# GPUOpen-Effects/FidelityFX-FSR

Hardware: NVIDIA H100
Metric: upscaled Mpixels/sec (EASU+RCAS) (higher is better)
Workload: dtype f16

## Files before the change

### fidelityfx-fsr_b200/csrc/fsr1_fused.cu

```cuda
#include "fsr1_easu_quad.cuh"
#include "fsr1_post.cuh"
#include "fsr1_rcas_math.cuh"

namespace fsr1 {

constexpr int kFBW = kQBW + 2;
constexpr int kFSW = kFBW - 2;
constexpr int kStripCells = 31;

struct FusedParams {
  ImgView in, out;
  int y0, y1;
  uint32_t sharp_h2;
  int n_strips;
  HaloSync sync = {};
};

template <int NW> struct FusedCfg {
  static constexpr int kCY = 2 * NW, kBH = kCY + 3, kSH = kCY + 1, kElems = kFBW * kBH;
  static constexpr int kPad = ((kElems * 8 + 127) / 128) * 128 / 8;
  static constexpr int kMidRows = 2 * kCY + 2;
};

template <int NW> struct __align__(128) FusedSmem {
  uint2 tile[2][FusedCfg<NW>::kPad];
  float4 S[kFSW * FusedCfg<NW>::kSH];
  uint4 mid[FusedCfg<NW>::kMidRows][32];
  float L[FusedCfg<NW>::kElems];
  uint64_t bar[2];
};

template <bool kIn> struct MidSink {
  uint4* top;
  bool zT, zB;
  uint32_t keep;
  __device__ __forceinline__ void put(bool bottom, __half2 oR, __half2 oG, __half2 oB) const {
    if (kIn) {
      top[bottom ? 32 : 0] = make_uint4(h22u(oR), h22u(oG), h22u(oB), 0u);
      return;
    }
    const uint32_t m = (bottom ? zB : zT) ? 0u : keep;
    top[bottom ? 32 : 0] = make_uint4(h22u(oR) & m, h22u(oG) & m, h22u(oB) & m, 0u);
  }
};

struct FusedStep { int tx, m0, n, ya, yb; };

template <int CY> struct FusedIter {
  int y0, y1, mfirst, mlast;
  int strip, strip_end, ma, mb, m;
  __device__ void init(const FusedParams& p, int cta, int ctas) {
    y0 = p.y0; y1 = p.y1;
    mfirst = (y0 - 2) >> 1;
    mlast = (y1 - 1) >> 1;
    const int S = p.n_strips, C = mlast - mfirst + 1;
    strip = strip_end = 0; ma = 0; mb = -1; m = 1;
    if (y1 <= y0) return;
    if (ctas < S) {
      strip = (int)((long long)S * cta / ctas);
      strip_end = (int)((long long)S * (cta + 1) / ctas);
      ma = mfirst; mb = mlast; m = ma;
      return;
    }
    const int s = (int)(((long long)(cta + 1) * S - 1) / ctas);
    const int g0 = (int)((long long)ctas * s / S), g = (int)((long long)ctas * (s + 1) / S) - g0, i = cta - g0;
    int T = (C + g - 1 + CY - 1) / CY;
    if (T < g) T = (C - 1 + CY - 2) / (CY - 1);
    const int a = (int)((long long)T * i / g), k = (int)((long long)T * (i + 1) / g) - a;
    const int ra = mfirst + CY * a - (i < a ? i : a);
    if (k == 0 || 2 * ra + 2 >= y1) return;
    ma = ra;
    mb = ma + CY * k - 1 < mlast ? ma + CY * k - 1 : mlast;
    strip = s; strip_end = s + 1; m = ma;
  }
  __device__ bool next(FusedStep& s) {
    if (m > mb) {
      if (++strip >= strip_end) return false;
      m = ma;
    }
    s.tx = strip; s.m0 = m;
    s.ya = 2 * ma + 2 > y0 ? 2 * ma + 2 : y0;
    s.yb = 2 * mb + 2 < y1 ? 2 * mb + 2 : y1;
    s.n = mb - m + 1 < CY ? mb - m + 1 : CY;
    m += s.n;
    return true;
  }
};

template <bool kIn, int NW, typename SO>
__device__ __forceinline__ void fused_step(FusedSmem<NW>& sm, const FusedParams& p, const FusedStep& cur, const uint2* tile, int dx,
                                           int k0, __half2 sharp, int lane, int warp, const PostParams* q) {
  constexpr int CY = FusedCfg<NW>::kCY;
  constexpr bool kPost = !std::is_void<SO>::value;
  const int n = cur.n;
#pragma unroll 1
  for (int q = 0; q < 2; q++) {
    const int r = warp + q * NW;
    if (!kIn && r >= n) break;
    const int pyT = 2 * (cur.m0 + r) + 1, pxA = 2 * (k0 + lane) + 1;
    MidSink<kIn> sink;
    sink.top = &sm.mid[2 * r + 2][lane];
    sink.zT = !kIn && (pyT < 0 || pyT >= p.out.h);
    sink.zB = !kIn && (pyT + 1 < 0 || pyT + 1 >= p.out.h);
    sink.keep = kIn ? 0xffffffffu
                    : ((pxA >= 0 && pxA < p.out.w) ? 0x0000ffffu : 0u) | ((pxA + 1 >= 0 && pxA + 1 < p.out.w) ? 0xffff0000u : 0u);
    quad_compute<MidSink<kIn>, kFBW, kFSW>(tile + dx, sm.S + dx, lane, r, true, true, sink);
  }
  __syncthreads();
  constexpr int kR = 2 * CY / NW;
  const int o_first = 2 * cur.m0 + warp * kR;
  const int i0 = warp * kR;
  const int lm = lane > 0 ? lane - 1 : 0;
  const int ox = 2 * (k0 + lane);
  const bool writer = lane >= 1 && (kIn || ox < p.out.w);
  const bool wtop = writer && (!kIn || o_first >= cur.ya);
  if constexpr (kPost) {
    auto mid_row = [&](int i, Row3& e, Row3& d, Row3& f) {
      const uint4 a = sm.mid[i][lm], c = sm.mid[i][lane];
      e.r = uh2(__byte_perm(a.x, c.x, 0x5432));
      e.g = uh2(__byte_perm(a.y, c.y, 0x5432));
      e.b = uh2(__byte_perm(a.z, c.z, 0x5432));
      d.r = uh2(a.x); d.g = uh2(a.y); d.b = uh2(a.z);
      f.r = uh2(c.x); f.g = uh2(c.y); f.b = uh2(c.z);
    };
    Row3 ea, eb, db, fb, ec, dc, fc;
    mid_row(i0, ea, dc, fc);
    mid_row(i0 + 1, eb, db, fb);
    unsigned char* dst = p.out.base + (long long)(o_first - p.out.row0) * p.out.pitch + (long long)ox * PostStore<SO>::kBytes;
    PostCursor pc;
    pc.init(*q, ox, o_first);
#pragma unroll
    for (int r = 0; r < kR; r++) {
      const int o = o_first + r;
      mid_row(i0 + r + 2, ec, dc, fc);
      if (kIn || (o >= cur.ya && o < cur.yb && o < 2 * cur.m0 + 2 * n)) {
        __half2 oR, oG, oB;
        rcas_pair<0>(ea, db, eb, fb, ec, sharp, oR, oG, oB);
        if (r >= 2 ? writer : wtop) post_pair<SO>(*q, pc, dst + (long long)r * p.out.pitch, ox, o, oR, oG, oB, 0x3c003c00u, kIn || ox + 1 < p.out.w);
      }
      pc.next_row(*q);
      ea = eb; eb = ec; db = dc; fb = fc;
    }
  } else {
    Row3 E[kR + 2], D[kR], Fv[kR];
#pragma unroll
    for (int r = 0; r < kR + 2; r++) {
      const uint4 a = sm.mid[i0 + r][lm], c = sm.mid[i0 + r][lane];
      E[r].r = uh2(__byte_perm(a.x, c.x, 0x5432));
      E[r].g = uh2(__byte_perm(a.y, c.y, 0x5432));
      E[r].b = uh2(__byte_perm(a.z, c.z, 0x5432));
      if (r >= 1 && r <= kR) {
        D[r - 1].r = uh2(a.x); D[r - 1].g = uh2(a.y); D[r - 1].b = uh2(a.z);
        Fv[r - 1].r = uh2(c.x); Fv[r - 1].g = uh2(c.y); Fv[r - 1].b = uh2(c.z);
      }
    }
    unsigned char* dst = p.out.base + (long long)(o_first - p.out.row0) * p.out.pitch + (long long)ox * 8;
#pragma unroll
    for (int r = 0; r < kR; r++) {
      const int o = o_first + r;
      if (kIn || (o >= cur.ya && o < cur.yb && o < 2 * cur.m0 + 2 * n)) {
        __half2 oR, oG, oB;
        rcas_pair<0>(E[r], D[r], E[r + 1], Fv[r], E[r + 2], sharp, oR, oG, oB);
        if (r >= 2 ? writer : wtop) {
          const uint4 w = pack_pair_half(oR, oG, oB, 0x3c003c00u);
          unsigned char* o8 = dst + (long long)r * p.out.pitch;
          if (kIn || ox + 1 < p.out.w) *reinterpret_cast<uint4*>(o8) = w;
          else *reinterpret_cast<uint2*>(o8) = make_uint2(w.x, w.y);
        }
      }
    }
  }
}

template <int NW, typename SO, bool kSrtmIn>
__device__ __forceinline__ void fused_body(const FusedParams p, const CUtensorMap& tmap, const PostParams* q) {
  using C = FusedCfg<NW>;
  constexpr int NT = NW * 32, CY = C::kCY;
  __shared__ FusedSmem<NW> sm;
  const int tid = threadIdx.x, lane = tid & 31, warp = tid >> 5;
  if (tid == 0) {
    mbar_init(&sm.bar[0], 1);
    mbar_init(&sm.bar[1], 1);
    mbar_fence_init();
  }
  __syncthreads();
  halo_sync_begin(p.sync);
  FusedIter<CY> iter;
  iter.init(p, blockIdx.x, gridDim.x);
  FusedStep cur, nxt;
  bool has = iter.next(cur);
  auto box_x = [](const FusedStep& s) { return (kStripCells * s.tx - 2) & ~1; };
  if (tid == 0 && has) {
    mbar_expect_tx(&sm.bar[0], C::kElems * 8u);
    tma_load_2d(sm.tile[0], &tmap, box_x(cur), cur.m0 - 1 - p.in.row0, &sm.bar[0]);
  }
  const __half2 sharp = uh2(p.sharp_h2);
  for (int it = 0; has; it++) {
    const int b = it & 1;
    const bool hasn = iter.next(nxt);
    if (tid == 0 && hasn) {
      fence_proxy_async();
      mbar_expect_tx(&sm.bar[b ^ 1], C::kElems * 8u);
      tma_load_2d(sm.tile[b ^ 1], &tmap, box_x(nxt), nxt.m0 - 1 - p.in.row0, &sm.bar[b ^ 1]);
    }
    uint2* tile = sm.tile[b];
    const int k0 = kStripCells * cur.tx - 1;
    const int gxe = box_x(cur), dx = (k0 - 1) - gxe;
    const int gy0 = cur.m0 - 1, n = cur.n;
    mbar_wait(&sm.bar[b], (it >> 1) & 1);
    if (gxe < 0 || gy0 < 0 || gxe + kFBW > p.in.w || gy0 + C::kBH > p.in.h) {
      clamp_fixup(tile, kFBW, kFBW, C::kBH, gxe, gy0, p.in.w, p.in.h, lane, warp, NW);
      fence_proxy_async();
      __syncthreads();
    }
    for (int i = tid; i < kFBW * (n + 3); i += NT) {
      uint2 c = tile[i];
      if (kSrtmIn) tile[i] = c = srtm_texel(c);
      sm.L[i] = texel_luma(c);
    }
    __syncthreads();
    for (int idx = tid; idx < kFSW * (n + 1); idx += NT) {
      const int j = idx / kFSW, i = idx - j * kFSW;
      const float* c = sm.L + (j + 1) * kFBW + (i + 1);
      sm.S[idx] = texel_terms(c[-kFBW], c[-1], c[0], c[1], c[kFBW]);
    }
    __syncthreads();
    const bool inside = k0 >= 0 && 2 * (k0 + 31) + 2 < p.out.w && cur.m0 >= 0 && 2 * (cur.m0 + CY) < p.out.h && n == CY &&
                        2 * cur.m0 + 2 >= cur.ya && 2 * (cur.m0 + CY) <= cur.yb;
    if (inside) fused_step<true, NW, SO>(sm, p, cur, tile, dx, k0, sharp, lane, warp, q);
    else fused_step<false, NW, SO>(sm, p, cur, tile, dx, k0, sharp, lane, warp, q);
    __syncthreads();
    if (n == CY && tid < 64) {
      const int rr = tid >> 5;
      sm.mid[rr][lane] = sm.mid[2 * CY + rr][lane];
    }
    cur = nxt;
    has = hasn;
  }
  halo_sync_end(p.sync);
}

template <int NW, int MINB, bool kSrtmIn = false>
__global__ void __launch_bounds__(NW * 32, MINB)
fused_h_quad2x_kernel(const FusedParams p, const __grid_constant__ CUtensorMap tmap) {
  fused_body<NW, void, kSrtmIn>(p, tmap, nullptr);
}

template <int NW, int MINB, typename SO, bool kSrtmIn = false>
__global__ void __launch_bounds__(NW * 32, MINB)
fused_h_quad2x_post_kernel(const FusedParams p, const __grid_constant__ CUtensorMap tmap, const __grid_constant__ PostParams q) {
  fused_body<NW, SO, kSrtmIn>(p, tmap, &q);
}

#ifndef FSR1_CPU_EMU
static cudaError_t fused_setup(const EasuParams& e, uint32_t sharp_h2, int out_align, CUtensorMap& tmap, FusedParams& p, int& per_sm,
                               long long& grid) {
  if (!(e.c0x == 0.5f && e.c0y == 0.5f && e.c0z == -0.25f && e.c0w == -0.25f)) return cudaErrorNotSupported;
  if ((reinterpret_cast<uintptr_t>(e.in.base) & 15) || (e.in.pitch & 15) || (reinterpret_cast<uintptr_t>(e.out.base) & (out_align - 1)) ||
      (e.out.pitch & (out_align - 1)))
    return cudaErrorNotSupported;
  constexpr int NW = 4;
  using C = FusedCfg<NW>;
  EncodeTiledFn encode = get_encode_fn();
  if (!encode) return cudaErrorNotSupported;
  const cuuint64_t dims[2] = {(cuuint64_t)e.in.w, (cuuint64_t)e.in.rows};
  const cuuint64_t strides[1] = {(cuuint64_t)e.in.pitch};
  const cuuint32_t box[2] = {(cuuint32_t)kFBW, (cuuint32_t)C::kBH};
  const cuuint32_t estr[2] = {1, 1};
  if (encode(&tmap, CU_TENSOR_MAP_DATA_TYPE_UINT64, 2, e.in.base, dims, strides, box, estr, CU_TENSOR_MAP_INTERLEAVE_NONE,
             CU_TENSOR_MAP_SWIZZLE_NONE, CU_TENSOR_MAP_L2_PROMOTION_L2_128B, CU_TENSOR_MAP_FLOAT_OOB_FILL_NONE) != CUDA_SUCCESS)
    return cudaErrorNotSupported;
  p.in = e.in; p.out = e.out; p.y0 = e.y0; p.y1 = e.y1; p.sharp_h2 = sharp_h2; p.sync = e.sync;
  p.n_strips = ((e.out.w + 1) / 2 + kStripCells - 1) / kStripCells;
  const long long units = (long long)p.n_strips * ((e.y1 - e.y0 + 1) / 2);
  if (p.sync.ready[0] || p.sync.ready[1]) per_sm = 6;
  grid = (long long)per_sm * sm_count();
  if (grid > (units + 7) / 8) grid = (units + 7) / 8;
  if (grid < 1) grid = 1;
  return cudaSuccess;
}

cudaError_t launch_fused_h(const EasuParams& e, uint32_t sharp_h2, int clamp, cudaStream_t s, const char** name, bool srtm_in) {
  if (clamp) return cudaErrorNotSupported;
  CUtensorMap tmap;
  FusedParams p;
  int per_sm = 7;
  long long grid = 0;
  const cudaError_t err = fused_setup(e, sharp_h2, 16, tmap, p, per_sm, grid);
  if (err != cudaSuccess) return err;
  if (srtm_in) {
    fused_h_quad2x_kernel<4, 7, true><<<(int)grid, 4 * 32, 0, s>>>(p, tmap);
    *name = per_sm == 7 ? "fused_easu_rcas_h_quad2x<4w,7/sm,tma2,strips,srtm_in>" : "fused_easu_rcas_h_quad2x<4w,6/sm,tma2,strips,srtm_in>";
  } else {
    fused_h_quad2x_kernel<4, 7><<<(int)grid, 4 * 32, 0, s>>>(p, tmap);
    *name = per_sm == 7 ? "fused_easu_rcas_h_quad2x<4w,7/sm,tma2,strips>" : "fused_easu_rcas_h_quad2x<4w,6/sm,tma2,strips>";
  }
  return cudaGetLastError();
}

constexpr int kPostPerSm = 6;

cudaError_t launch_fused_h_post(const EasuParams& e, uint32_t sharp_h2, const PostParams& q, int out_format, cudaStream_t s,
                                const char** name, bool srtm_in) {
  CUtensorMap tmap;
  FusedParams p;
  int per_sm = kPostPerSm;
  long long grid = 0;
  const cudaError_t err = fused_setup(e, sharp_h2, out_format == 1 ? 16 : 8, tmap, p, per_sm, grid);
  if (err != cudaSuccess) return err;
  switch (out_format * 2 + (srtm_in ? 1 : 0)) {
    case 2:
      fused_h_quad2x_post_kernel<4, kPostPerSm, __half><<<(int)grid, 4 * 32, 0, s>>>(p, tmap, q);
      *name = "fused_easu_rcas_h_quad2x<4w,6/sm,tma2,strips,post,rgba16f>";
      break;
    case 6:
      fused_h_quad2x_post_kernel<4, kPostPerSm, Unorm8><<<(int)grid, 4 * 32, 0, s>>>(p, tmap, q);
      *name = "fused_easu_rcas_h_quad2x<4w,6/sm,tma2,strips,post,rgba8>";
      break;
    case 8:
      fused_h_quad2x_post_kernel<4, kPostPerSm, Unorm10><<<(int)grid, 4 * 32, 0, s>>>(p, tmap, q);
      *name = "fused_easu_rcas_h_quad2x<4w,6/sm,tma2,strips,post,rgb10a2>";
      break;
    case 3:
      fused_h_quad2x_post_kernel<4, kPostPerSm, __half, true><<<(int)grid, 4 * 32, 0, s>>>(p, tmap, q);
      *name = "fused_easu_rcas_h_quad2x<4w,6/sm,tma2,strips,post,rgba16f,srtm_in>";
      break;
    case 7:
      fused_h_quad2x_post_kernel<4, kPostPerSm, Unorm8, true><<<(int)grid, 4 * 32, 0, s>>>(p, tmap, q);
      *name = "fused_easu_rcas_h_quad2x<4w,6/sm,tma2,strips,post,rgba8,srtm_in>";
      break;
    case 9:
      fused_h_quad2x_post_kernel<4, kPostPerSm, Unorm10, true><<<(int)grid, 4 * 32, 0, s>>>(p, tmap, q);
      *name = "fused_easu_rcas_h_quad2x<4w,6/sm,tma2,strips,post,rgb10a2,srtm_in>";
      break;
    default: return cudaErrorNotSupported;
  }
  return cudaGetLastError();
}
#endif

}
```

Before: 105,600.

## Raise fused EASU+RCAS tile height to three cell rows per warp

Makes the number of cell rows each warp handles a template parameter, set by default to three instead of two, so each CTA tile covers more output rows and the vertical halo (loads, luma and terms rows) is amortized over more work. The RCAS output loop is unified into a single rolling-row form, with a reduced unroll for the post-processing path. The launches now request the maximum shared-memory carveout so the larger tiles still fit 7 (or 6) CTAs per SM, and static asserts check this. The cost is more shared memory and longer per-step work per CTA, which may reduce load balance or occupancy.

```diff
diff --git a/fidelityfx-fsr_b200/csrc/fsr1_fused.cu b/fidelityfx-fsr_b200/csrc/fsr1_fused.cu
--- a/fidelityfx-fsr_b200/csrc/fsr1_fused.cu
+++ b/fidelityfx-fsr_b200/csrc/fsr1_fused.cu
@@ -5,8 +5,9 @@
 namespace fsr1 {
 
 constexpr int kFBW = kQBW + 2;
-constexpr int kFSW = kFBW - 2;
+constexpr int kFSW = 34;
 constexpr int kStripCells = 31;
+constexpr int kFusedCPW = 3;
 
 struct FusedParams {
   ImgView in, out;
@@ -16,17 +17,18 @@
   HaloSync sync = {};
 };
 
-template <int NW> struct FusedCfg {
-  static constexpr int kCY = 2 * NW, kBH = kCY + 3, kSH = kCY + 1, kElems = kFBW * kBH;
+template <int NW, int CPW = kFusedCPW> struct FusedCfg {
+  static constexpr int kCY = CPW * NW, kBH = kCY + 3, kSH = kCY + 1, kElems = kFBW * kBH;
   static constexpr int kPad = ((kElems * 8 + 127) / 128) * 128 / 8;
   static constexpr int kMidRows = 2 * kCY + 2;
 };
 
-template <int NW> struct __align__(128) FusedSmem {
-  uint2 tile[2][FusedCfg<NW>::kPad];
-  float4 S[kFSW * FusedCfg<NW>::kSH];
-  uint4 mid[FusedCfg<NW>::kMidRows][32];
-  float L[FusedCfg<NW>::kElems];
+template <int NW, int CPW> struct __align__(128) FusedSmem {
+  using C = FusedCfg<NW, CPW>;
+  uint2 tile[2][C::kPad];
+  float4 S[kFSW * C::kSH];
+  uint4 mid[C::kMidRows][32];
+  float L[C::kElems];
   uint64_t bar[2];
 };
 
@@ -87,14 +89,13 @@
   }
 };
 
-template <bool kIn, int NW, typename SO>
-__device__ __forceinline__ void fused_step(FusedSmem<NW>& sm, const FusedParams& p, const FusedStep& cur, const uint2* tile, int dx,
+template <bool kIn, int NW, int CPW, typename SO>
+__device__ __forceinline__ void fused_step(FusedSmem<NW, CPW>& sm, const FusedParams& p, const FusedStep& cur, const uint2* tile, int dx,
                                            int k0, __half2 sharp, int lane, int warp, const PostParams* q) {
-  constexpr int CY = FusedCfg<NW>::kCY;
   constexpr bool kPost = !std::is_void<SO>::value;
   const int n = cur.n;
 #pragma unroll 1
-  for (int q = 0; q < 2; q++) {
+  for (int q = 0; q < CPW; q++) {
     const int r = warp + q * NW;
     if (!kIn && r >= n) break;
     const int pyT = 2 * (cur.m0 + r) + 1, pxA = 2 * (k0 + lane) + 1;
@@ -107,76 +108,56 @@
     quad_compute<MidSink<kIn>, kFBW, kFSW>(tile + dx, sm.S + dx, lane, r, true, true, sink);
   }
   __syncthreads();
-  constexpr int kR = 2 * CY / NW;
+  constexpr int kR = 2 * CPW;
   const int o_first = 2 * cur.m0 + warp * kR;
   const int i0 = warp * kR;
   const int lm = lane > 0 ? lane - 1 : 0;
   const int ox = 2 * (k0 + lane);
   const bool writer = lane >= 1 && (kIn || ox < p.out.w);
   const bool wtop = writer && (!kIn || o_first >= cur.ya);
-  if constexpr (kPost) {
-    auto mid_row = [&](int i, Row3& e, Row3& d, Row3& f) {
-      const uint4 a = sm.mid[i][lm], c = sm.mid[i][lane];
-      e.r = uh2(__byte_perm(a.x, c.x, 0x5432));
-      e.g = uh2(__byte_perm(a.y, c.y, 0x5432));
-      e.b = uh2(__byte_perm(a.z, c.z, 0x5432));
-      d.r = uh2(a.x); d.g = uh2(a.y); d.b = uh2(a.z);
-      f.r = uh2(c.x); f.g = uh2(c.y); f.b = uh2(c.z);
-    };
-    Row3 ea, eb, db, fb, ec, dc, fc;
-    mid_row(i0, ea, dc, fc);
-    mid_row(i0 + 1, eb, db, fb);
-    unsigned char* dst = p.out.base + (long long)(o_first - p.out.row0) * p.out.pitch + (long long)ox * PostStore<SO>::kBytes;
-    PostCursor pc;
-    pc.init(*q, ox, o_first);
-#pragma unroll
-    for (int r = 0; r < kR; r++) {
-      const int o = o_first + r;
-      mid_row(i0 + r + 2, ec, dc, fc);
-      if (kIn || (o >= cur.ya && o < cur.yb && o < 2 * cur.m0 + 2 * n)) {
-        __half2 oR, oG, oB;
-        rcas_pair<0>(ea, db, eb, fb, ec, sharp, oR, oG, oB);
-        if (r >= 2 ? writer : wtop) post_pair<SO>(*q, pc, dst + (long long)r * p.out.pitch, ox, o, oR, oG, oB, 0x3c003c00u, kIn || ox + 1 < p.out.w);
-      }
-      pc.next_row(*q);
-      ea = eb; eb = ec; db = dc; fb = fc;
-    }
-  } else {
-    Row3 E[kR + 2], D[kR], Fv[kR];
-#pragma unroll
-    for (int r = 0; r < kR + 2; r++) {
-      const uint4 a = sm.mid[i0 + r][lm], c = sm.mid[i0 + r][lane];
-      E[r].r = uh2(__byte_perm(a.x, c.x, 0x5432));
-      E[r].g = uh2(__byte_perm(a.y, c.y, 0x5432));
-      E[r].b = uh2(__byte_perm(a.z, c.z, 0x5432));
-      if (r >= 1 && r <= kR) {
-        D[r - 1].r = uh2(a.x); D[r - 1].g = uh2(a.y); D[r - 1].b = uh2(a.z);
-        Fv[r - 1].r = uh2(c.x); Fv[r - 1].g = uh2(c.y); Fv[r - 1].b = uh2(c.z);
-      }
-    }
-    unsigned char* dst = p.out.base + (long long)(o_first - p.out.row0) * p.out.pitch + (long long)ox * 8;
-#pragma unroll
-    for (int r = 0; r < kR; r++) {
-      const int o = o_first + r;
-      if (kIn || (o >= cur.ya && o < cur.yb && o < 2 * cur.m0 + 2 * n)) {
-        __half2 oR, oG, oB;
-        rcas_pair<0>(E[r], D[r], E[r + 1], Fv[r], E[r + 2], sharp, oR, oG, oB);
-        if (r >= 2 ? writer : wtop) {
+  auto mid_row = [&](int i, Row3& e, Row3& d, Row3& f) {
+    const uint4 a = sm.mid[i][lm], c = sm.mid[i][lane];
+    e.r = uh2(__byte_perm(a.x, c.x, 0x5432));
+    e.g = uh2(__byte_perm(a.y, c.y, 0x5432));
+    e.b = uh2(__byte_perm(a.z, c.z, 0x5432));
+    d.r = uh2(a.x); d.g = uh2(a.y); d.b = uh2(a.z);
+    f.r = uh2(c.x); f.g = uh2(c.y); f.b = uh2(c.z);
+  };
+  Row3 ea, eb, db, fb, ec, dc, fc;
+  mid_row(i0, ea, dc, fc);
+  mid_row(i0 + 1, eb, db, fb);
+  unsigned char* dst = p.out.base + (long long)(o_first - p.out.row0) * p.out.pitch + (long long)ox * PostStore<SO>::kBytes;
+  PostCursor pc;
+  if constexpr (kPost) pc.init(*q, ox, o_first);
+  constexpr int kUnroll = kPost ? 2 : kR;
+#pragma unroll kUnroll
+  for (int r = 0; r < kR; r++) {
+    const int o = o_first + r;
+    mid_row(i0 + r + 2, ec, dc, fc);
+    if (kIn || (o >= cur.ya && o < cur.yb && o < 2 * cur.m0 + 2 * n)) {
+      __half2 oR, oG, oB;
+      rcas_pair<0>(ea, db, eb, fb, ec, sharp, oR, oG, oB);
+      if (r >= 2 ? writer : wtop) {
+        unsigned char* o8 = dst + (long long)r * p.out.pitch;
+        if constexpr (kPost) {
+          post_pair<SO>(*q, pc, o8, ox, o, oR, oG, oB, 0x3c003c00u, kIn || ox + 1 < p.out.w);
+        } else {
           const uint4 w = pack_pair_half(oR, oG, oB, 0x3c003c00u);
-          unsigned char* o8 = dst + (long long)r * p.out.pitch;
           if (kIn || ox + 1 < p.out.w) *reinterpret_cast<uint4*>(o8) = w;
           else *reinterpret_cast<uint2*>(o8) = make_uint2(w.x, w.y);
         }
       }
     }
-  }
-}
-
-template <int NW, typename SO, bool kSrtmIn>
+    if constexpr (kPost) pc.next_row(*q);
+    ea = eb; eb = ec; db = dc; fb = fc;
+  }
+}
+
+template <int NW, int CPW, typename SO, bool kSrtmIn>
 __device__ __forceinline__ void fused_body(const FusedParams p, const CUtensorMap& tmap, const PostParams* q) {
-  using C = FusedCfg<NW>;
+  using C = FusedCfg<NW, CPW>;
   constexpr int NT = NW * 32, CY = C::kCY;
-  __shared__ FusedSmem<NW> sm;
+  __shared__ FusedSmem<NW, CPW> sm;
   const int tid = threadIdx.x, lane = tid & 31, warp = tid >> 5;
   if (tid == 0) {
     mbar_init(&sm.bar[0], 1);
@@ -227,8 +208,8 @@
     __syncthreads();
     const bool inside = k0 >= 0 && 2 * (k0 + 31) + 2 < p.out.w && cur.m0 >= 0 && 2 * (cur.m0 + CY) < p.out.h && n == CY &&
                         2 * cur.m0 + 2 >= cur.ya && 2 * (cur.m0 + CY) <= cur.yb;
-    if (inside) fused_step<true, NW, SO>(sm, p, cur, tile, dx, k0, sharp, lane, warp, q);
-    else fused_step<false, NW, SO>(sm, p, cur, tile, dx, k0, sharp, lane, warp, q);
+    if (inside) fused_step<true, NW, CPW, SO>(sm, p, cur, tile, dx, k0, sharp, lane, warp, q);
+    else fused_step<false, NW, CPW, SO>(sm, p, cur, tile, dx, k0, sharp, lane, warp, q);
     __syncthreads();
     if (n == CY && tid < 64) {
       const int rr = tid >> 5;
@@ -240,19 +221,42 @@
   halo_sync_end(p.sync);
 }
 
-template <int NW, int MINB, bool kSrtmIn = false>
+template <int NW, int MINB, bool kSrtmIn = false, int CPW = kFusedCPW>
 __global__ void __launch_bounds__(NW * 32, MINB)
 fused_h_quad2x_kernel(const FusedParams p, const __grid_constant__ CUtensorMap tmap) {
-  fused_body<NW, void, kSrtmIn>(p, tmap, nullptr);
-}
-
-template <int NW, int MINB, typename SO, bool kSrtmIn = false>
+  fused_body<NW, CPW, void, kSrtmIn>(p, tmap, nullptr);
+}
+
+template <int NW, int MINB, typename SO, bool kSrtmIn = false, int CPW = kFusedCPW>
 __global__ void __launch_bounds__(NW * 32, MINB)
 fused_h_quad2x_post_kernel(const FusedParams p, const __grid_constant__ CUtensorMap tmap, const __grid_constant__ PostParams q) {
-  fused_body<NW, SO, kSrtmIn>(p, tmap, &q);
+  fused_body<NW, CPW, SO, kSrtmIn>(p, tmap, &q);
 }
 
 #ifndef FSR1_CPU_EMU
+constexpr int kPostPerSm = 6;
+
+constexpr size_t kFusedSmemPerCta = sizeof(FusedSmem<4, kFusedCPW>) + 1024;
+static_assert(7 * kFusedSmemPerCta <= 228 * 1024, "the fused kernel's shared memory must admit 7 CTAs per SM");
+static_assert(kPostPerSm * kFusedSmemPerCta <= 228 * 1024, "the fused post kernels' shared memory must admit 6 CTAs per SM");
+
+template <auto K> static cudaError_t max_shared_carveout() {
+  static bool done[64] = {};
+  int dev = 0;
+  if (cudaGetDevice(&dev) != cudaSuccess || dev < 0 || dev >= 64) dev = -1;
+  if (dev >= 0 && done[dev]) return cudaSuccess;
+  const cudaError_t e = cudaFuncSetAttribute(K, cudaFuncAttributePreferredSharedMemoryCarveout, (int)cudaSharedmemCarveoutMaxShared);
+  if (e == cudaSuccess && dev >= 0) done[dev] = true;
+  return e;
+}
+
+template <auto K, typename... A> static cudaError_t fused_launch(long long grid, cudaStream_t s, const A&... args) {
+  const cudaError_t e = max_shared_carveout<K>();
+  if (e != cudaSuccess) return e;
+  K<<<(int)grid, 4 * 32, 0, s>>>(args...);
+  return cudaGetLastError();
+}
+
 static cudaError_t fused_setup(const EasuParams& e, uint32_t sharp_h2, int out_align, CUtensorMap& tmap, FusedParams& p, int& per_sm,
                                long long& grid) {
   if (!(e.c0x == 0.5f && e.c0y == 0.5f && e.c0z == -0.25f && e.c0w == -0.25f)) return cudaErrorNotSupported;
@@ -289,16 +293,12 @@
   const cudaError_t err = fused_setup(e, sharp_h2, 16, tmap, p, per_sm, grid);
   if (err != cudaSuccess) return err;
   if (srtm_in) {
-    fused_h_quad2x_kernel<4, 7, true><<<(int)grid, 4 * 32, 0, s>>>(p, tmap);
     *name = per_sm == 7 ? "fused_easu_rcas_h_quad2x<4w,7/sm,tma2,strips,srtm_in>" : "fused_easu_rcas_h_quad2x<4w,6/sm,tma2,strips,srtm_in>";
-  } else {
-    fused_h_quad2x_kernel<4, 7><<<(int)grid, 4 * 32, 0, s>>>(p, tmap);
-    *name = per_sm == 7 ? "fused_easu_rcas_h_quad2x<4w,7/sm,tma2,strips>" : "fused_easu_rcas_h_quad2x<4w,6/sm,tma2,strips>";
-  }
-  return cudaGetLastError();
-}
-
-constexpr int kPostPerSm = 6;
+    return fused_launch<fused_h_quad2x_kernel<4, 7, true>>(grid, s, p, tmap);
+  }
+  *name = per_sm == 7 ? "fused_easu_rcas_h_quad2x<4w,7/sm,tma2,strips>" : "fused_easu_rcas_h_quad2x<4w,6/sm,tma2,strips>";
+  return fused_launch<fused_h_quad2x_kernel<4, 7>>(grid, s, p, tmap);
+}
 
 cudaError_t launch_fused_h_post(const EasuParams& e, uint32_t sharp_h2, const PostParams& q, int out_format, cudaStream_t s,
                                 const char** name, bool srtm_in) {
@@ -310,32 +310,25 @@
   if (err != cudaSuccess) return err;
   switch (out_format * 2 + (srtm_in ? 1 : 0)) {
     case 2:
-      fused_h_quad2x_post_kernel<4, kPostPerSm, __half><<<(int)grid, 4 * 32, 0, s>>>(p, tmap, q);
       *name = "fused_easu_rcas_h_quad2x<4w,6/sm,tma2,strips,post,rgba16f>";
-      break;
+      return fused_launch<fused_h_quad2x_post_kernel<4, kPostPerSm, __half>>(grid, s, p, tmap, q);
     case 6:
-      fused_h_quad2x_post_kernel<4, kPostPerSm, Unorm8><<<(int)grid, 4 * 32, 0, s>>>(p, tmap, q);
       *name = "fused_easu_rcas_h_quad2x<4w,6/sm,tma2,strips,post,rgba8>";
-      break;
+      return fused_launch<fused_h_quad2x_post_kernel<4, kPostPerSm, Unorm8>>(grid, s, p, tmap, q);
     case 8:
-      fused_h_quad2x_post_kernel<4, kPostPerSm, Unorm10><<<(int)grid, 4 * 32, 0, s>>>(p, tmap, q);
       *name = "fused_easu_rcas_h_quad2x<4w,6/sm,tma2,strips,post,rgb10a2>";
-      break;
+      return fused_launch<fused_h_quad2x_post_kernel<4, kPostPerSm, Unorm10>>(grid, s, p, tmap, q);
     case 3:
-      fused_h_quad2x_post_kernel<4, kPostPerSm, __half, true><<<(int)grid, 4 * 32, 0, s>>>(p, tmap, q);
       *name = "fused_easu_rcas_h_quad2x<4w,6/sm,tma2,strips,post,rgba16f,srtm_in>";
-      break;
+      return fused_launch<fused_h_quad2x_post_kernel<4, kPostPerSm, __half, true>>(grid, s, p, tmap, q);
     case 7:
-      fused_h_quad2x_post_kernel<4, kPostPerSm, Unorm8, true><<<(int)grid, 4 * 32, 0, s>>>(p, tmap, q);
       *name = "fused_easu_rcas_h_quad2x<4w,6/sm,tma2,strips,post,rgba8,srtm_in>";
-      break;
+      return fused_launch<fused_h_quad2x_post_kernel<4, kPostPerSm, Unorm8, true>>(grid, s, p, tmap, q);
     case 9:
-      fused_h_quad2x_post_kernel<4, kPostPerSm, Unorm10, true><<<(int)grid, 4 * 32, 0, s>>>(p, tmap, q);
       *name = "fused_easu_rcas_h_quad2x<4w,6/sm,tma2,strips,post,rgb10a2,srtm_in>";
-      break;
+      return fused_launch<fused_h_quad2x_post_kernel<4, kPostPerSm, Unorm10, true>>(grid, s, p, tmap, q);
     default: return cudaErrorNotSupported;
   }
-  return cudaGetLastError();
 }
 #endif
 
```

New measurement: 90150, median of 6. 0.854x the previous value.
